# davidea97/Fisher-Nerf-customized

Measured on AMD Instinct MI355X. Metric: candidate-views/sec, higher is better.
Workload: dtype f32

## Files before the change

### fisher-nerf-customized_amd/csrc/fisher_rast.hip

```cpp
#include <hip/hip_runtime.h>
#include <hip/hip_fp16.h>
#include <stdint.h>
#include <stdio.h>
#include <stdlib.h>
#include <string.h>
#include "fr_math.h"
#include "../../include/fisher_rast.h"
#include "fr_internal.h"

#define FR_THREADS 256
#define FR_G_MAX 32
#define FR_MAX_LDS_TILES 4096
#define FR_PART_MIN_DEFAULT 2048
#define FR_SORT_SMALL_KEYS 2048
#define FR_SORT_MID_KEYS 4096
#define FR_SORT_BIG_KEYS 16384
#define FR_VC_MAX 16
#define FR_BATCH 256
#define FR_BWD_BATCH 128

#include <vector>
#include <utility>
static thread_local char g_err[512] = "";
#if defined(FR_ABLATE) || defined(FR_LOOPSTATS)
// ... 33 lines not shown

struct FrParams {
	int P, V, W, H;
	uint32_t gx, gy;
	int T;
	int G;
	float tanfovx, tanfovy, focal_x, focal_y, mod;
	int D, M;
	const float* bg; const float* view; const float* proj; const float* campos;
	const float* w2c;
	const float* means3D; const float* colors; const float* shs; const float* opac;
	const float* scales; const float* rots;
	const float* cov3D;
	float* cov3D_out;
	int* radii;
	FrSplat* splat;
	float* rgb;
	uint8_t* clamped;
	uint32_t* tile_cnt; uint32_t* tile_off; uint32_t* tile_fill;
	uint64_t* keys; long long key_capacity;
	uint32_t* blk_base;
	uint32_t* big_list;
	uint32_t* view_work;
	uint32_t* view_perm;
	int* status;
	int* vis_count;
	int* num_rendered;
	struct FrVisEntry* vis_list;
	uint32_t* vis_n;
	int VC;
	uint32_t tile_cap;
	uint32_t small_max;
	const uint32_t* order;
	int legacy_sort;
	int prefiltered;
	int ablate;
};
#ifdef FR_ABLATE
#define FR_ABL(x) x
#else
#define FR_ABL(x)
#endif

__device__ __forceinline__ float wave_sum(float v)
{
#pragma unroll
// ... 1137 lines not shown
	{
		uint4 en[NB];
#pragma unroll
		for (int b = 0; b < NB; b++)
		{
			const uint32_t e = e0 + b * FR_THREADS + tid;
			en[b] = e < n ? list[e] : make_uint4(0u, 0u, 0u, 0u);
		}
#pragma unroll
		for (int b = 0; b < NB; b++)
		{
			const uint64_t key = ((uint64_t)en[b].y << 32) | en[b].x;
			const uint32_t x0 = en[b].z & 0xffffu, y0 = en[b].z >> 16, x1 = en[b].w & 0xffffu, y1 = en[b].w >> 16;
			for (uint32_t y = y0; y < y1; y++)
				for (uint32_t x = x0; x < x1; x++)
				{
					const uint32_t t = y * p.gx + x;
					p.keys[s_base[t] + atomicAdd(&s_cnt[t], 1u)] = key;
				}
		}
	}
}

__device__ __forceinline__ void fr_tile_of_block(const FrParams& p, uint32_t& tile, int& v)
{
	const uint32_t L = blockIdx.x;
	if ((p.V & 7) == 0)
	{
		const uint32_t xcd = L & 7u, q = L >> 3;
		v = (int)((q / (uint32_t)p.T) * 8u + xcd);
		if (p.view_perm) v = (int)p.view_perm[v];
		tile = q % (uint32_t)p.T;
	}
	else
	{
		v = (int)(L / (uint32_t)p.T);
		tile = L % (uint32_t)p.T;
	}
}

__device__ __forceinline__ void fr_cx(uint64_t& lo, uint64_t& hi)
{
	const uint64_t a = lo, b = hi;
	const bool sw = a > b;
	lo = sw ? b : a; hi = sw ? a : b;
}
template <typename KeyPtr>
__device__ __forceinline__ uint64_t fr_ldk(KeyPtr keys, uint32_t i, uint32_t n) { return i < n ? keys[i] : ~0ull; }
template <typename KeyPtr>
// ... 233 lines not shown
		}
	}
}

template <int K, int NW>
__device__ __forceinline__ void fr_sort_wg_segment(uint64_t* sk, uint64_t* __restrict__ gk, uint32_t n, int tid)
{
	static_assert(NW == 4 || NW == 16, "4 or 16 waves");
	constexpr int RUN = 64 * K;
	const int lane = tid & 63;
	const int w = __builtin_amdgcn_readfirstlane(tid >> 6);
	const uint32_t base = (uint32_t)(w * RUN);
	uint64_t key[K];
#pragma unroll
	for (int r = 0; r < K; r++) { const uint32_t i = base + (uint32_t)(lane * K + r); key[r] = i < n ? gk[i] : ~0ull; }
	uint32_t n_pad = 1;
	while (n_pad < n) n_pad <<= 1;
	fr_wave_stages<K, 6 + FrLog2<K>::value>(key, n_pad, lane);
	fr_wg_stages<K, NW, (NW == 4 ? 2 : 4)>(key, sk, n_pad, w, lane);
#pragma unroll
	for (int r = 0; r < K; r++) { const uint32_t i = base + (uint32_t)(lane * K + r); if (i < n) gk[i] = key[r]; }
}

__global__ __launch_bounds__(FR_THREADS) void k_sort_tiles(FrParams p)
{
	if (p.status[1]) return;
	__shared__ uint64_t skeys[FR_SORT_SMALL_KEYS];
	const int tid = threadIdx.x;
	uint32_t tile; int v;
	fr_tile_of_block(p, tile, v);
	const size_t vt = (size_t)v * p.T + tile;
	const uint32_t n = p.tile_cnt[vt];
	if (n < 2 || n > p.small_max) return;
	uint64_t* gk = p.keys + p.tile_off[vt];
#ifdef FR_AB
	if (p.legacy_sort)
	{
		for (uint32_t i = tid; i < n; i += FR_THREADS) skeys[i] = gk[i];
		__syncthreads();
		fr_bitonic(skeys, n, tid, FR_THREADS);
		for (uint32_t i = tid; i < n; i += FR_THREADS) gk[i] = skeys[i];
		return;
	}
#endif
	if (n <= 512u)
	{
		if (tid >= 64) return;
		if (n <= 64u) fr_sort_wave_segment<1>(gk, n, tid);
		else if (n <= 128u) fr_sort_wave_segment<2>(gk, n, tid);
		else if (n <= 256u) fr_sort_wave_segment<4>(gk, n, tid);
		else fr_sort_wave_segment<8>(gk, n, tid);
		return;
	}
	if (n <= 1024u) fr_sort_wg_segment<4, 4>(skeys, gk, n, tid);
	else fr_sort_wg_segment<8, 4>(skeys, gk, n, tid);
}

#define FR_PART_SAMPLE 512
#define FR_PART_MAXP 64
__global__ __launch_bounds__(FR_THREADS) void k_sort_part(FrParams p, uint32_t part_max)
{
	__shared__ uint64_t skeys[FR_SORT_SMALL_KEYS];
	__shared__ uint64_t s_piv[FR_PART_MAXP];
	__shared__ uint32_t s_cnt[FR_PART_MAXP], s_off[FR_PART_MAXP], s_cur[FR_PART_MAXP];
	__shared__ uint32_t s_next;
	if (p.status[1]) return;
	const int tid = threadIdx.x, lane = tid & 63;
	const uint32_t count = p.big_list[0];
	for (uint32_t b = blockIdx.x; b < count; b += gridDim.x)
	{
		const size_t vt = p.big_list[16 + b];
		const uint32_t n = p.tile_cnt[vt];
		if (n > part_max) continue;
		uint64_t* gk = p.keys + p.tile_off[vt];
		const uint32_t n_al = (n + 63u) & ~63u;
		uint64_t* tmp = gk + n_al;
		const uint32_t NP = n <= 1280u ? 4u : n <= 2560u ? 8u : n <= 5120u ? 16u : n <= 10240u ? 32u : 64u;
		__syncthreads();
		if (tid < FR_PART_MAXP) { s_cnt[tid] = 0u; s_cur[tid] = 0u; }
		if (tid == 0) s_next = 0u;
		if (tid < 64)
		{
			uint64_t key[8];
#pragma unroll
			for (int r = 0; r < 8; r++) key[r] = gk[(uint32_t)(((uint64_t)(uint32_t)(lane * 8 + r) * n) >> 9)];
			fr_wave_stages<8, 9>(key, (uint32_t)FR_PART_SAMPLE, lane);
			const uint32_t step = 64u / NP;
			if (((uint32_t)lane % step) == 0u && lane > 0) s_piv[(uint32_t)lane / step] = key[0];
		}
		__syncthreads();
		auto part_of = [&](uint64_t k) -> uint32_t {
			uint32_t lo = 0u;
			for (uint32_t stepw = NP >> 1; stepw > 0u; stepw >>= 1)
			{
				const uint32_t mid = lo + stepw;
				if (s_piv[mid] <= k) lo = mid;
			}
			return lo;
		};
		constexpr int KB = 8;
		for (uint32_t i0 = 0; i0 < n; i0 += KB * FR_THREADS)
		{
			uint64_t k[KB];
#pragma unroll
			for (int r = 0; r < KB; r++) { const uint32_t i = i0 + r * FR_THREADS + tid; k[r] = i < n ? gk[i] : ~0ull; }
#pragma unroll
			for (int r = 0; r < KB; r++) { const uint32_t i = i0 + r * FR_THREADS + tid; if (i < n) atomicAdd(&s_cnt[part_of(k[r])], 1u); }
		}
		__syncthreads();
		if (tid == 0)
		{
			uint32_t run = 0;
			for (uint32_t q = 0; q < NP; q++) { s_off[q] = run; run += s_cnt[q]; }
		}
		__syncthreads();
		for (uint32_t i0 = 0; i0 < n; i0 += KB * FR_THREADS)
		{
			uint64_t k[KB];
#pragma unroll
			for (int r = 0; r < KB; r++) { const uint32_t i = i0 + r * FR_THREADS + tid; k[r] = i < n ? gk[i] : ~0ull; }
#pragma unroll
			for (int r = 0; r < KB; r++)
			{
				const uint32_t i = i0 + r * FR_THREADS + tid;
				if (i < n) { const uint32_t q = part_of(k[r]); tmp[s_off[q] + atomicAdd(&s_cur[q], 1u)] = k[r]; }
			}
		}
		__syncthreads();
		for (;;)
		{
			uint32_t q = 0;
			if (lane == 0) q = atomicAdd(&s_next, 1u);
			q = (uint32_t)__builtin_amdgcn_readfirstlane((int)q);
			if (q >= NP) break;
			const uint32_t c = s_cnt[q];
			uint64_t* pk = tmp + s_off[q];
			if (c < 2u || c > 512u) continue;
			if (c <= 64u) fr_sort_wave_segment<1>(pk, c, lane);
			else if (c <= 128u) fr_sort_wave_segment<2>(pk, c, lane);
			else if (c <= 256u) fr_sort_wave_segment<4>(pk, c, lane);
			else fr_sort_wave_segment<8>(pk, c, lane);
		}
		__syncthreads();
		for (uint32_t q = 0; q < NP; q++)
		{
			const uint32_t c = s_cnt[q];
			if (c <= 512u) continue;
			uint64_t* pk = tmp + s_off[q];
			if (c <= 1024u) fr_sort_wg_segment<4, 4>(skeys, pk, c, tid);
			else if (c <= (uint32_t)FR_SORT_SMALL_KEYS) fr_sort_wg_segment<8, 4>(skeys, pk, c, tid);
			else fr_bitonic(pk, c, tid, FR_THREADS);
			__syncthreads();
		}
		if (tid == 0) p.tile_off[vt] += n_al;
	}
}

__global__ __launch_bounds__(FR_THREADS) void k_sort_mid_tiles(FrParams p, uint32_t part_max)
{
	if (p.status[1]) return;
	__shared__ uint64_t skeys[FR_SORT_MID_KEYS];
	const int tid = threadIdx.x;
	const uint32_t count = p.big_list[0];
	for (uint32_t b = blockIdx.x; b < count; b += gridDim.x)
	{
		const size_t vt = p.big_list[16 + b];
		const uint32_t n = p.tile_cnt[vt];
		if (n > (uint32_t)FR_SORT_MID_KEYS || n <= part_max) continue;
		uint64_t* gk = p.keys + p.tile_off[vt];
		__syncthreads();
#ifdef FR_AB
		if (p.legacy_sort)
		{
			for (uint32_t i = tid; i < n; i += FR_THREADS) skeys[i] = gk[i];
			__syncthreads();
			fr_bitonic(skeys, n, tid, FR_THREADS);
			for (uint32_t i = tid; i < n; i += FR_THREADS) gk[i] = skeys[i];
// ... 4388 lines not shown
	FrSideStream& ss = sides[which];
	int dev = -1;
	(void)hipGetDevice(&dev);
	if (ss.device != dev)
	{
		if (ss.ok) { (void)hipEventDestroy(ss.fork); (void)hipEventDestroy(ss.join); (void)hipStreamDestroy(ss.stream); }
#ifdef FR_AB
		static const int tile_prio = fr_env_int("FR_TILE_PRIO");
#else
		constexpr int tile_prio = 0;
#endif
		int lo = 0, hi = 0;
		(void)hipDeviceGetStreamPriorityRange(&lo, &hi);
		const int prio = (which == 2 && tile_prio > 0) ? lo : (which == 2 && tile_prio < 0) ? hi : 0;
		ss.ok = hipStreamCreateWithPriority(&ss.stream, hipStreamNonBlocking, prio) == hipSuccess
		     && hipEventCreateWithFlags(&ss.fork, hipEventDisableTiming) == hipSuccess
		     && hipEventCreateWithFlags(&ss.join, hipEventDisableTiming) == hipSuccess;
		ss.device = dev;
		(void)hipGetLastError();
	}
	return ss;
}

struct FrJoinGuard {
	hipStream_t s; FrSideStream* side[2] = { nullptr, nullptr }; int n = 0;
	explicit FrJoinGuard(hipStream_t caller) : s(caller) {}
	void forked(FrSideStream* ss) { side[n++] = ss; }
	int join()
	{
		int rc = FR_OK;
		for (int i = 0; i < n; i++)
		{
			if (hipEventRecord(side[i]->join, side[i]->stream) != hipSuccess || hipStreamWaitEvent(s, side[i]->join, 0) != hipSuccess)
				rc = fr_fail(FR_ELAUNCH, "side stream join failed");
		}
		n = 0;
		return rc;
	}
	~FrJoinGuard() { if (n) { char keep[sizeof(g_err)]; memcpy(keep, g_err, sizeof(keep)); (void)join(); memcpy(g_err, keep, sizeof(keep)); } }
};

struct FrScorerPlan { int columns; bool form_a; FrRecordArgs ra; bool skip_pack = false; bool general = false; bool pose = false; bool view_identity = false; };
template <int C> __global__ void k_pack_static(FrParams p, const float* __restrict__ H_inv, float* __restrict__ packed, float4* __restrict__ mt, float4* __restrict__ grp);
template <int C, bool LIST, bool FORM_A> __global__ void k_fisher_records(FrParams p, FrRecordArgs ra);

static int fr_bin_pipeline(FrParams& p, const fr_gaussians* g, hipStream_t s, const FrScorerPlan* plan = nullptr)
{
	int rc;
	const int P = p.P;
	{
		FrZeroer z;
		z.add(p.tile_cnt, (size_t)p.V * p.T * 4); z.add(p.status, 16); z.add(p.big_list, 64);
		if (p.view_work) z.add(p.view_work, (size_t)p.V * 4);
		if (p.vis_count) z.add(p.vis_count, (size_t)p.V * 4);
		if (p.num_rendered && p.vis_list != nullptr && p.T <= FR_MAX_LDS_TILES) z.add(p.num_rendered, (size_t)p.V * 4);
		z.launch(s);
	}
	const bool multi = p.vis_list != nullptr && p.T <= FR_MAX_LDS_TILES;
	if (g->cov3D_precomp) p.cov3D = g->cov3D_precomp;
	else if (plan && multi) p.cov3D = nullptr;
	else
	{
		hipLaunchKernelGGL(k_cov3d, dim3((P + FR_THREADS - 1) / FR_THREADS), dim3(FR_THREADS), 0, s, P, g->scales, p.mod, g->rotations, p.cov3D_out);
		if ((rc = fr_check_launch("k_cov3d"))) return rc;
		p.cov3D = p.cov3D_out;
	}
	p.G = multi ? fr_pick_G_views(P) : fr_pick_G(P, p.V);
	p.VC = fr_pick_VC(p.T);
	const int per_block = FR_THREADS * p.G;
	dim3 gridP((P + per_block - 1) / per_block, p.V);
	const size_t hist_lds = p.T <= FR_MAX_LDS_TILES ? (size_t)p.T * 4 : 16;
	if (plan && !plan->skip_pack)
	{
		const float* shared_hinv = plan->ra.hinv_stride ? nullptr : plan->ra.H_inv;
		dim3 gp((P + FR_THREADS - 1) / FR_THREADS);
// ... 58 lines not shown
	if ((rc = fr_check_launch("k_scan_tiles"))) return rc;
	if (multi && p.tile_cap) {  }
	else if (multi) hipLaunchKernelGGL(k_scatter_vis, gridP, dim3(FR_THREADS), 2 * hist_lds, s, p);
	else hipLaunchKernelGGL(k_scatter_keys, gridP, dim3(FR_THREADS), 2 * hist_lds, s, p);
	if ((rc = fr_check_launch("k_scatter_keys"))) return rc;
	if (plan && !multi)
	{
		FrSideStream& s2 = fr_side_stream(1);
		const bool forked2 = s2.ok && hipEventRecord(s2.fork, s) == hipSuccess && hipStreamWaitEvent(s2.stream, s2.fork, 0) == hipSuccess;
		hipStream_t rs = forked2 ? s2.stream : s;
		if (plan->form_a) hipLaunchKernelGGL((k_fisher_records<4, false, true>), gridP, dim3(FR_THREADS), 0, rs, p, plan->ra);
		else if (plan->columns == 4) hipLaunchKernelGGL((k_fisher_records<4, false, false>), gridP, dim3(FR_THREADS), 0, rs, p, plan->ra);
		else hipLaunchKernelGGL((k_fisher_records<11, false, false>), gridP, dim3(FR_THREADS), 0, rs, p, plan->ra);
		if (forked2) joins.forked(&s2);
		if ((rc = fr_check_launch("k_fisher_records"))) return rc;
	}
	FrSideStream& side = fr_side_stream();
	const bool part_all = p.tile_cap >= 32768u && fr_debug_mode() != 32;
	const bool want_fork = fr_debug_mode() != 7 && (!multi || p.V >= 8) && !part_all;
	const bool forked = want_fork && side.ok && hipEventRecord(side.fork, s) == hipSuccess && hipStreamWaitEvent(side.stream, side.fork, 0) == hipSuccess;
	const int big_blocks = p.T * p.V < 256 ? p.T * p.V : 256;
	if (forked) joins.forked(&side);
	uint32_t part_max = 0;
	if (p.tile_cap >= 2u * (uint32_t)FR_SORT_SMALL_KEYS + 128u && fr_debug_mode() != 32)
	{
		part_max = p.tile_cap / 2u - 64u;
		if (part_max > 16320u) part_max = 16320u;
	}
	hipLaunchKernelGGL(k_sort_big_tiles, dim3(big_blocks), dim3(1024), 0, forked ? side.stream : s, p, part_max);
	if ((rc = fr_check_launch("k_sort_big_tiles"))) return rc;
	const int mid_blocks = p.T * p.V < 2048 ? p.T * p.V : 2048;
	hipLaunchKernelGGL(k_sort_tiles, dim3(p.T * p.V), dim3(FR_THREADS), 0, s, p);
	if ((rc = fr_check_launch("k_sort_tiles"))) return rc;
	if (part_max)
	{
		hipLaunchKernelGGL(k_sort_part, dim3(mid_blocks), dim3(FR_THREADS), 0, s, p, part_max);
		if ((rc = fr_check_launch("k_sort_part"))) return rc;
	}
	if (part_max < (uint32_t)FR_SORT_MID_KEYS)
	{
		hipLaunchKernelGGL(k_sort_mid_tiles, dim3(mid_blocks), dim3(FR_THREADS), 0, s, p, part_max);
		if ((rc = fr_check_launch("k_sort_mid_tiles"))) return rc;
	}
	return joins.join();
}

static void fr_carve_single(FrParams& p, const FrLayout& L, char* geom, char* bin, char* img)
{
	p.splat = (FrSplat*)(geom + L.splat);
	p.cov3D_out = (float*)(geom + L.cov3D);
	p.rgb = (float*)(geom + L.rgb);
	p.clamped = (uint8_t*)(geom + L.clamped);
	p.tile_cnt = (uint32_t*)(img + L.tile_cnt);
	p.tile_off = (uint32_t*)(img + L.tile_off);
	p.tile_fill = (uint32_t*)(img + L.tile_fill);
	p.status = (int*)(img + L.status);
	p.big_list = (uint32_t*)(img + L.big_list);
	p.blk_base = p.T <= FR_MAX_LDS_TILES ? (uint32_t*)(img + L.blk_base) : nullptr;
	p.keys = (uint64_t*)(bin + L.keys);
}
// ... 382 lines not shown
		b.only_flagged = fallback; b.u_only = 1;
		if (sr) hipLaunchKernelGGL((k_backward_tile<true, false>), grid, block, 0, s, p, b);
		else hipLaunchKernelGGL((k_backward_tile<false, false>), grid, block, 0, s, p, b);
		if ((rc = fr_check_launch("k_backward_tile(flagged)"))) return rc;
	}
	b.dL_dmean2D = dL_dmeans2D; b.dL_dmean2D_b = dL_dmeans2D_features;
	b.dL_dcolors = dL_dcolors; b.colors = g->colors_precomp;
	dim3 gp((P + FR_THREADS - 1) / FR_THREADS);
	if (sr) hipLaunchKernelGGL((k_backward_finish<true, false>), gp, block, 0, s, p, b, (float*)nullptr);
	else hipLaunchKernelGGL((k_backward_finish<false, false>), gp, block, 0, s, p, b, (float*)nullptr);
	return fr_check_launch("k_backward_finish");
}

#ifdef FR_AB
static int fr_debug_mode()
{
	static const int mode = fr_env_int("FR_DEBUG_MODE");
	return mode;
}
#endif

#define FR_MAX_GROUPS 4
struct FrFisherLayout {
	size_t radii, vis_n, splat, recq, slot_idx, packed, mt, grp, big_list, view_work, view_perm, blk_base, cov3D, tile_cnt, tile_off, tile_fill, tile_scores, w2c_inv, status, keys, fallback, seg_T, seg_C, seg_X, seg_list, total;
	size_t PV;
};
static FrFisherLayout fr_fisher_layout(int64_t P, int64_t W, int64_t H, int64_t V, int64_t max_rendered, int columns)
{
	FrFisherLayout L;
	const int64_t T = ((W + 15) / 16) * ((H + 15) / 16);
	size_t o = 0;
	const size_t nblk_v = (size_t)((P + FR_THREADS * fr_pick_G_views(P) - 1) / (FR_THREADS * fr_pick_G_views(P)));
	L.radii = o; o = fr_align(o + (size_t)V * nblk_v * (size_t)(FR_THREADS * fr_pick_G_views(P)) * sizeof(FrVisEntry));
	L.vis_n = o; o = fr_align(o + (size_t)V * nblk_v * 4);
	L.PV = nblk_v * (size_t)(FR_THREADS * fr_pick_G_views(P));
	const size_t VPV = (size_t)V * (L.PV > (size_t)P ? L.PV : (size_t)P);
	L.splat = o; o = fr_align(o + VPV * sizeof(FrSplat));
	L.recq = o; o = fr_align(o + VPV * (columns == 11 ? 208 : 112));
	L.slot_idx = o; o = fr_align(o + VPV * 4);
	L.packed = o; o = fr_align(o + (size_t)P * 4 * (size_t)(columns == 11 ? 32 : 16));
	L.mt = o; o = fr_align(o + (size_t)P * 16);
	L.grp = o; o = fr_align(o + (size_t)((P + FR_THREADS - 1) / FR_THREADS) * 32);
	L.big_list = o; o = fr_align(o + (size_t)(V * T) * 4 + 64 * FR_MAX_GROUPS);
	L.view_work = o; o = fr_align(o + (size_t)V * 4);
	L.view_perm = o; o = fr_align(o + (size_t)V * 4);
	L.blk_base = o; o = fr_align(o + (size_t)V * (size_t)fr_preprocess_blocks(P, V) * (size_t)T * 4);
	L.cov3D = o; o = fr_align(o + (size_t)P * 24);
	L.tile_cnt = o; o = fr_align(o + (size_t)(V * T) * 4);
	L.tile_off = o; o = fr_align(o + (size_t)(V * T) * 4);
	L.tile_fill = o; o = fr_align(o + (size_t)(V * T) * 4);
	L.tile_scores = o; o = fr_align(o + (size_t)(V * T) * 4);
	L.w2c_inv = o; o = fr_align(o + (size_t)V * 64);
	L.status = o; o = fr_align(o + 64);
	const size_t R = (size_t)(max_rendered > 0 ? max_rendered : 1);
	L.keys = o; o = fr_align(o + R * 8);
	L.fallback = o; o = fr_align(o + (size_t)(V * T));
	const size_t seg_tiles = (size_t)(V * T <= FR_SEG_TILES ? V * T : 0);
	L.seg_T = o; o = fr_align(o + FR_SEG_PER_TILE * seg_tiles * FR_THREADS * 4);
	L.seg_C = o; o = fr_align(o + FR_SEG_PER_TILE * seg_tiles * FR_THREADS * 8);
	L.seg_X = o; o = fr_align(o + seg_tiles * FR_THREADS * 8);
	L.seg_list = o; o = fr_align(o + (FR_SEG_PER_TILE * seg_tiles + 1) * 4);
	L.total = o;
	return L;
}

extern "C" int fr_fisher_workspace_layout(int32_t P, int32_t W, int32_t H, int32_t n_views, int64_t max_rendered, int32_t columns, size_t o[8])
{
	if (P < 0 || W <= 0 || H <= 0 || n_views <= 0 || max_rendered < 0 || (columns != 4 && columns != 11) || !o)
		return fr_fail(FR_EINVAL, "fr_fisher_workspace_layout: bad argument");
	const FrFisherLayout L = fr_fisher_layout(P, W, H, n_views, max_rendered, columns);
	o[0] = L.tile_cnt; o[1] = L.tile_off; o[2] = L.keys; o[3] = L.splat; o[4] = L.recq; o[5] = L.tile_scores; o[6] = L.status; o[7] = L.vis_n;
	return FR_OK;
}

extern "C" int fr_init(void)
{
	if (!fr_side_stream(0).ok || !fr_side_stream(1).ok || !fr_side_stream(2).ok) return fr_fail(FR_ELAUNCH, "fr_init: could not create the side streams");
	return FR_OK;
}

extern "C" size_t fr_fisher_workspace_bytes(int32_t P, int32_t W, int32_t H, int32_t n_views, int64_t max_rendered, int32_t columns)
{
	if (P < 0 || W <= 0 || H <= 0 || n_views <= 0 || max_rendered < 0 || (columns != 4 && columns != 11)) return 0;
	return fr_fisher_layout(P, W, H, n_views, max_rendered, columns).total;
}

static void fr_launch_fisher_v3(FrParams& p, FrFisherArgs f, float4* recq, hipStream_t s)
{
	hipEvent_t ev0 = nullptr, ev1 = nullptr;
	if (g_prof_on)
	{
		(void)hipEventCreate(&ev0); (void)hipEventCreate(&ev1);
		(void)hipEventRecord(ev0, s);
	}
// ... 120 lines not shown
	if (!workspace || workspace_bytes < L.total) return fr_fail(FR_ENOSPACE, "fr_fisher_views: workspace smaller than fr_fisher_workspace_bytes()");
	char* ws = (char*)workspace;
	FrParams p;
	fr_fill_params(p, cfg, g, V);
	p.prefiltered = 0;
	p.w2c = fc->w2c;
	if (fc->poses_are_c2w)
	{
		float* inv = (float*)(ws + L.w2c_inv);
		hipLaunchKernelGGL(k_invert_poses, dim3((V + 63) / 64), dim3(64), 0, s, V, fc->w2c, inv);
		if ((rc = fr_check_launch("k_invert_poses"))) return rc;
		p.w2c = inv;
	}
	p.radii = (int*)(ws + L.radii);
	p.vis_list = (FrVisEntry*)(ws + L.radii);
	p.vis_n = (uint32_t*)(ws + L.vis_n);
	p.splat = (FrSplat*)(ws + L.splat);
	p.cov3D_out = (float*)(ws + L.cov3D);
	p.tile_cnt = (uint32_t*)(ws + L.tile_cnt);
	p.tile_off = (uint32_t*)(ws + L.tile_off);
	p.tile_fill = (uint32_t*)(ws + L.tile_fill);
	p.status = (int*)(ws + L.status);
	p.big_list = (uint32_t*)(ws + L.big_list);
	const bool deal = (V & 7) == 0 && V <= 1024 && fr_debug_mode() != 27;
	p.view_work = deal ? (uint32_t*)(ws + L.view_work) : nullptr;
	p.view_perm = deal ? (uint32_t*)(ws + L.view_perm) : nullptr;
	p.blk_base = (uint32_t*)(ws + L.blk_base);
	p.keys = (uint64_t*)(ws + L.keys);
	p.key_capacity = max_rendered;
	if (fc->tile_capacity < 0) return fr_fail(FR_EINVAL, "fr_fisher_views: negative tile_capacity");
	if (fc->tile_capacity > 0)
	{
		const long long need = (long long)V * p.T * (long long)fc->tile_capacity;
		if (need > max_rendered || need >= (1ll << 32)) return fr_fail(FR_EINVAL, "fr_fisher_views: n_views * tiles * tile_capacity exceeds max_rendered (or 2^32)");
		const long long nblk_c = (P + FR_THREADS * fr_pick_G_views(P) - 1) / (FR_THREADS * fr_pick_G_views(P));
		const bool slots_fit = nblk_c * FR_THREADS * fr_pick_G_views(P) < (1ll << 28);
		if (p.gx <= 255u && p.gy <= 63u && slots_fit && fr_debug_mode() != 8 && fr_debug_mode() != 24 && fr_debug_mode() != 20) p.tile_cap = (uint32_t)fc->tile_capacity;
	}
	p.vis_count = fc->out_vis_count;
	p.num_rendered = fc->out_num_rendered;
	FrFisherArgs f;
	f.dL = fc->dL_dpix;
	f.dL_img = fc->dL_dpix_image; f.dL_stride = fc->dL_image_view_stride;
	f.H_inv = fc->H_inv; f.hinv_stride = fc->H_inv_view_stride;
	f.out_H = fc->out_H; f.outH_stride = fc->out_H_view_stride;
	f.tile_scores = (float*)(ws + L.tile_scores);
// ... 43 lines not shown
	static thread_local hipEvent_t front_done[FR_MAX_GROUPS] = { nullptr, nullptr, nullptr, nullptr };
	const size_t nblk_v = (size_t)((P + FR_THREADS * fr_pick_G_views(P) - 1) / (FR_THREADS * fr_pick_G_views(P)));
	const size_t cap_v = (size_t)(FR_THREADS * fr_pick_G_views(P));
	const size_t rec_view = compact ? L.PV : (size_t)P;
	struct TileJoin {
		hipStream_t s; FrSideStream* side; bool on;
		~TileJoin() { if (on) { (void)hipEventRecord(side->join, side->stream); (void)hipStreamWaitEvent(s, side->join, 0); } }
	} tile_join{ s, &tside, false };
	for (int gi = 0; gi < n_groups; gi++)
	{
		const int per = n_groups > 1 ? ((V / n_groups + 7) / 8) * 8 : V;
		const int v0 = gi * per, Vg = (gi == n_groups - 1) ? V - v0 : per;
		if (Vg <= 0) break;
		FrParams pg = p;
		pg.V = Vg;
		pg.w2c = p.w2c + 16 * (size_t)v0;
		pg.radii = p.radii ? (int*)((char*)p.radii + (size_t)v0 * nblk_v * cap_v * sizeof(FrVisEntry)) : nullptr;
		pg.vis_list = p.vis_list + (size_t)v0 * nblk_v * cap_v;
		pg.vis_n = p.vis_n + (size_t)v0 * nblk_v;
		pg.splat = p.splat + (size_t)v0 * rec_view;
		pg.tile_cnt = p.tile_cnt + (size_t)v0 * p.T; pg.tile_off = p.tile_off + (size_t)v0 * p.T; pg.tile_fill = p.tile_fill + (size_t)v0 * p.T;
		pg.status = p.status + 4 * gi;
		pg.big_list = p.big_list + (size_t)v0 * p.T + 16 * gi;
		if (p.view_perm && (Vg & 7) == 0) { pg.view_work = p.view_work + v0; pg.view_perm = p.view_perm + v0; }
		else { pg.view_work = nullptr; pg.view_perm = nullptr; }
		pg.blk_base = p.blk_base + (size_t)v0 * (size_t)fr_preprocess_blocks(P, V) * (size_t)p.T;
		pg.tile_cap = p.tile_cap;
		const long long k0 = (long long)((__int128)max_rendered * v0 / V), k1 = (long long)((__int128)max_rendered * (v0 + Vg) / V);
		pg.keys = p.keys + k0; pg.key_capacity = k1 - k0;
		pg.vis_count = p.vis_count ? p.vis_count + v0 : nullptr;
		pg.num_rendered = p.num_rendered ? p.num_rendered + v0 : nullptr;
		FrScorerPlan pl = plan;
		pl.skip_pack = gi > 0 || (fc->reuse_static != 0 && compact);
		if (pl.ra.hinv_stride) pl.ra.H_inv = plan.ra.H_inv + (size_t)v0 * plan.ra.hinv_stride;
		pl.ra.recq = plan.ra.recq + (size_t)v0 * rec_view * 4;
		if (pl.ra.comp) pl.ra.comp = plan.ra.comp + (size_t)v0 * L.PV * rstride;
		if (pl.ra.slot_idx) pl.ra.slot_idx = plan.ra.slot_idx + (size_t)v0 * L.PV;
		FrFisherArgs fg = f;
		fg.recA = f.recA + (size_t)v0 * f.ab_view; fg.recQ = f.recQ + (size_t)v0 * f.q_view;
		if (f.slot_idx) fg.slot_idx = f.slot_idx + (size_t)v0 * f.slot_view;
		fg.tile_scores = f.tile_scores + (size_t)v0 * p.T;
		if (f.H_inv && f.hinv_stride) fg.H_inv = f.H_inv + (size_t)v0 * f.hinv_stride;
		if (f.out_H && f.outH_stride) fg.out_H = f.out_H + (size_t)v0 * f.outH_stride;
		if (f.dL_img && f.dL_stride) fg.dL_img = f.dL_img + (size_t)v0 * f.dL_stride;

		if ((rc = fr_bin_pipeline(pg, g, s, (v3 || v3h || v3g) ? &pl : nullptr))) return rc;
// ... 87 lines not shown
		return fr_fail(FR_ENOSPACE, "fr_fisher_pose_views: workspace smaller than fr_fisher_pose_workspace_bytes()");
	char* ws = (char*)workspace;
	FrParams p;
	fr_fill_params(p, cfg, g, V);
	p.prefiltered = 0;
	p.w2c = fc->w2c;
	if (fc->poses_are_c2w)
	{
		float* inv = (float*)(ws + L.w2c_inv);
		hipLaunchKernelGGL(k_invert_poses, dim3((V + 63) / 64), dim3(64), 0, s, V, fc->w2c, inv);
		if ((rc = fr_check_launch("k_invert_poses"))) return rc;
		p.w2c = inv;
	}
	p.radii = (int*)(ws + L.radii);
	p.vis_list = (FrVisEntry*)(ws + L.radii);
	p.vis_n = (uint32_t*)(ws + L.vis_n);
	p.splat = (FrSplat*)(ws + L.splat);
	p.cov3D_out = (float*)(ws + L.cov3D);
	p.tile_cnt = (uint32_t*)(ws + L.tile_cnt);
	p.tile_off = (uint32_t*)(ws + L.tile_off);
	p.tile_fill = (uint32_t*)(ws + L.tile_fill);
	p.status = (int*)(ws + L.status);
	p.big_list = (uint32_t*)(ws + L.big_list);
	const bool deal = (V & 7) == 0 && V <= 1024;
	p.view_work = deal ? (uint32_t*)(ws + L.view_work) : nullptr;
	p.view_perm = deal ? (uint32_t*)(ws + L.view_perm) : nullptr;
	p.blk_base = (uint32_t*)(ws + L.blk_base);
	p.keys = (uint64_t*)(ws + L.keys);
	p.key_capacity = max_rendered;
	if (fc->tile_capacity > 0)
	{
		const long long nblk_c = (P + FR_THREADS * fr_pick_G_views(P) - 1) / (FR_THREADS * fr_pick_G_views(P));
		const bool slots_fit = nblk_c * FR_THREADS * fr_pick_G_views(P) < (1ll << 28);
		if (p.gx <= 255u && p.gy <= 63u && slots_fit) p.tile_cap = (uint32_t)fc->tile_capacity;
	}
	(void)fr_plan_views_c(p.T, fr_pick_VC(p.T), p.tile_cap);
	p.vis_count = fc->out_vis_count;
	p.num_rendered = fc->out_num_rendered;
	p.order = fc->order;
	constexpr int rstride = FrRecStride<4, 3>::value;
	FrScorerPlan plan;
	plan.columns = 4;
	plan.form_a = false;
	plan.pose = true;
	plan.ra.H_inv = nullptr; plan.ra.hinv_stride = 0;
	plan.ra.packed = (const float*)(ws + L.packed); plan.ra.recq = (float4*)(ws + L.recq);
// ... 467 lines not shown
```

### fisher-nerf-customized_amd/fisher_rast/_lib.py

```python
import ctypes
import os

_HERE = os.path.dirname(os.path.abspath(__file__))
SO_PATH = os.environ.get("FISHER_RAST_SO", os.path.join(_HERE, "libfisher_rast.so"))

FR_OK, FR_EINVAL, FR_ELAUNCH, FR_ENOSPACE = 0, 1, 2, 3

_f32p = ctypes.c_void_p


class RasterCfg(ctypes.Structure):
    _fields_ = [
        ("P", ctypes.c_int32),
        ("image_height", ctypes.c_int32),
        ("image_width", ctypes.c_int32),
        ("tanfovx", ctypes.c_float),
        ("tanfovy", ctypes.c_float),
        ("scale_modifier", ctypes.c_float),
        ("sh_degree", ctypes.c_int32),
        ("sh_coeffs", ctypes.c_int32),
        ("prefiltered", ctypes.c_int32),
        ("bg", _f32p),
        ("viewmatrix", _f32p),
        ("projmatrix", _f32p),
# ... 30 lines not shown
        ("dL_image_view_stride", ctypes.c_int64),
        ("tile_capacity", ctypes.c_int32),
        ("poses_are_c2w", ctypes.c_int32),
        ("reuse_static", ctypes.c_int32),
        ("order", ctypes.c_void_p),
        ("view_is_identity", ctypes.c_int32),
    ]


class OccCfg(ctypes.Structure):
    _fields_ = [
        ("grid_w", ctypes.c_int32),
        ("grid_h", ctypes.c_int32),
        ("cell_size", ctypes.c_float),
        ("center_x", ctypes.c_float),
        ("center_z", ctypes.c_float),
        ("height_lower", ctypes.c_float),
        ("height_upper", ctypes.c_float),
        ("far_distance", ctypes.c_float),
    ]


EXPORTS = (
    "fr_version", "fr_last_error", "fr_build_id", "fr_init", "fr_fisher_workspace_layout", "fr_workspace_bytes", "fr_workspace_layout", "fr_mark_visible",
    "fr_forward", "fr_backward", "fr_backward_scratch_bytes", "fr_backward_ws", "fr_forward_pair", "fr_forward_features", "fr_backward_pair", "fr_backward_pair_scratch_bytes", "fr_backward_pair_ws", "fr_fisher_workspace_bytes", "fr_fisher_views",
    "fr_fisher_pose_workspace_bytes", "fr_fisher_pose_workspace_layout", "fr_fisher_pose_views",
    "fr_densify_stats", "fr_densify_masks", "fr_prune_mask", "fr_knn_workspace_bytes", "fr_knn_dist2", "fr_spatial_order_workspace_bytes", "fr_spatial_order", "fr_profile_enable", "fr_profile_fetch",
    "fr_occ_workspace_bytes", "fr_occ_update", "fr_occ_freespace", "fr_occ_frontiers", "fr_occ_erode", "fr_occ_cells_of",
    "fr_occ_ring_candidates", "fr_occ_free_candidates",
)

_lib = None

_CSRC = os.path.join(os.path.dirname(_HERE), "csrc")
_INCLUDE = os.path.join(os.path.dirname(os.path.dirname(_HERE)), "include")
SOURCES = [os.path.join(_CSRC, n) for n in ("fisher_rast.hip", "fisher_occ.hip", "fr_math.h", "fr_internal.h")] + \
          [os.path.join(_INCLUDE, n) for n in ("fisher_rast.h", "fisher_occ.h")]


def source_hash():
    import hashlib
    h = hashlib.sha256()
    for f in SOURCES:
        if not os.path.exists(f):
            return None
        h.update(open(f, "rb").read())
    return h.hexdigest()[:16]


class FisherRastError(RuntimeError):
    pass


def load():
    global _lib
    if _lib is not None:
        return _lib
    if not os.path.exists(SO_PATH):
        raise FisherRastError(
            f"{SO_PATH} is missing: the HIP extension has not been built "
            "(run `python -c \"import __graft_entry__ as g; g.build()\"` at the repo root). "
            "There is no CPU fallback for this path.")
    import torch
    lib = ctypes.CDLL(SO_PATH)
    for name in EXPORTS:
        if not hasattr(lib, name):
            raise FisherRastError(f"{SO_PATH} does not export {name}")
    lib.fr_version.restype = ctypes.c_int
    lib.fr_last_error.restype = ctypes.c_char_p
    lib.fr_build_id.restype = ctypes.c_char_p
    lib.fr_init.restype = ctypes.c_int
    lib.fr_fisher_workspace_layout.restype = ctypes.c_int
    lib.fr_fisher_workspace_layout.argtypes = [ctypes.c_int32, ctypes.c_int32, ctypes.c_int32, ctypes.c_int32,
                                               ctypes.c_int64, ctypes.c_int32, ctypes.POINTER(ctypes.c_size_t)]
    want = source_hash()
    got = lib.fr_build_id().decode().split(":")[-1]
    if "FISHER_RAST_SO" not in os.environ and want is not None and got != want:
        raise FisherRastError(f"{SO_PATH} was built from other sources (build id {got}, sources {want}): "
                              "run `python -c \"import __graft_entry__ as g; g.build()\"`")
    lib.fr_workspace_bytes.restype = ctypes.c_int
    lib.fr_workspace_bytes.argtypes = [ctypes.c_int32, ctypes.c_int32, ctypes.c_int32, ctypes.c_int64,
                                       ctypes.POINTER(ctypes.c_size_t)]
    lib.fr_workspace_layout.restype = ctypes.c_int
    lib.fr_workspace_layout.argtypes = [ctypes.c_int32, ctypes.c_int32, ctypes.c_int32, ctypes.c_int64,
                                        ctypes.POINTER(ctypes.c_size_t)]
    lib.fr_mark_visible.restype = ctypes.c_int
    lib.fr_mark_visible.argtypes = [ctypes.c_int32, _f32p, _f32p, _f32p, ctypes.c_void_p, ctypes.c_void_p]
    lib.fr_forward.restype = ctypes.c_int
    lib.fr_forward.argtypes = [ctypes.POINTER(RasterCfg), ctypes.POINTER(Gaussians),
                               ctypes.c_void_p, ctypes.c_void_p, ctypes.c_int64, ctypes.c_void_p,
                               _f32p, _f32p, ctypes.c_void_p, ctypes.c_void_p, ctypes.c_void_p]
    lib.fr_backward.restype = ctypes.c_int
    lib.fr_backward.argtypes = [ctypes.POINTER(RasterCfg), ctypes.POINTER(Gaussians), ctypes.c_void_p,
                                ctypes.c_void_p, ctypes.c_void_p, ctypes.c_void_p,
                                _f32p, ctypes.c_int32] + [_f32p] * 9 + [ctypes.c_void_p]
    lib.fr_backward_scratch_bytes.restype = ctypes.c_size_t
    lib.fr_backward_scratch_bytes.argtypes = [ctypes.c_int32] * 4 + [ctypes.c_int64]
# ... 88 lines not shown
```

### include/fisher_rast.h

```cpp
#ifndef FISHER_RAST_H_INCLUDED
#define FISHER_RAST_H_INCLUDED

#include <stddef.h>
#include <stdint.h>

#ifdef __cplusplus
extern "C" {
#endif

#define FR_VERSION 100

enum {
	FR_OK = 0,
	FR_EINVAL = 1,
	FR_ELAUNCH = 2,
	FR_ENOSPACE = 3
};

#define FR_STATUS_WORDS 4

typedef void* fr_stream_t;

typedef struct fr_raster_cfg {
	int32_t P;
// ... 84 lines not shown
	const float* w2c;
	const float* H_inv;
	int64_t H_inv_view_stride;
	float* out_scores;
	float* out_H;
	int64_t out_H_view_stride;
	int32_t* out_vis_count;
	int32_t* out_num_rendered;
	const float* dL_dpix_image;
	int64_t dL_image_view_stride;
	int32_t tile_capacity;
	int32_t poses_are_c2w;
	int32_t reuse_static;
	const uint32_t* order;
	int32_t view_is_identity;
} fr_fisher_cfg;

size_t fr_spatial_order_workspace_bytes(int32_t P);
int fr_spatial_order(int32_t P, const float* means3D, uint32_t* order_out, void* workspace, size_t workspace_bytes, fr_stream_t stream);

size_t fr_fisher_workspace_bytes(int32_t P, int32_t W, int32_t H, int32_t n_views, int64_t max_rendered, int32_t columns);
int fr_fisher_workspace_layout(int32_t P, int32_t W, int32_t H, int32_t n_views, int64_t max_rendered, int32_t columns,
                               size_t offsets[8]);

int fr_fisher_views(const fr_raster_cfg* cfg, const fr_gaussians* g, const fr_fisher_cfg* cfg_f,
                    void* workspace, size_t workspace_bytes, int64_t max_rendered,
                    int32_t* status, fr_stream_t stream);

size_t fr_fisher_pose_workspace_bytes(int32_t P, int32_t W, int32_t H, int32_t n_views, int64_t max_rendered);
int fr_fisher_pose_workspace_layout(int32_t P, int32_t W, int32_t H, int32_t n_views, int64_t max_rendered, size_t offsets[9]);
int fr_fisher_pose_views(const fr_raster_cfg* cfg, const fr_gaussians* g, const fr_fisher_cfg* cfg_f, float* out_pose_H,
                         void* workspace, size_t workspace_bytes, int64_t max_rendered, int32_t* status, fr_stream_t stream);


int fr_densify_stats(int32_t P, const int32_t* radii, const float* grad_means2D, float* max_2D_radius,
                     float* means2D_gradient_accum, float* denom, uint8_t* seen, fr_stream_t stream);

int fr_densify_masks(int32_t P, const float* means2D_gradient_accum, const float* denom, const float* log_scales,
                     int32_t scale_cols, float grad_thresh, float clone_max_scale, float split_min_scale,
                     uint8_t* to_clone, uint8_t* to_split, fr_stream_t stream);

int fr_prune_mask(int32_t P, const float* logit_opacities, const float* log_scales, int32_t scale_cols,
                  float opacity_thresh, float big_thresh, uint8_t* to_remove, fr_stream_t stream);


size_t fr_knn_workspace_bytes(int32_t P);
// ... 12 lines not shown
```

Baseline: 46060.

## Merge short-tile sort into partition kernel and sort partitions in separate wave kernel

The separate short-tile sort launch is folded into the partition kernel: extra blocks beyond a CU-scaled count sort the short tiles. Mid-size partitions are no longer sorted serially by the waves of the block that partitioned them. Their offsets are appended to a global list and sorted one per wave in a new k_sort_parts kernel, spreading the work across the whole GPU. Pivot sampling now uses all four waves, and the partition prefix sum uses a wave scan. The cost is an extra kernel launch, extra workspace for the partition list, and global atomics.

```diff
diff --git a/fisher-nerf-customized_amd/csrc/fisher_rast.hip b/fisher-nerf-customized_amd/csrc/fisher_rast.hip
--- a/fisher-nerf-customized_amd/csrc/fisher_rast.hip
+++ b/fisher-nerf-customized_amd/csrc/fisher_rast.hip
@@ -79,6 +79,7 @@
 	uint32_t* blk_base;
 	uint32_t* big_list;
 	uint32_t* view_work;
+	uint32_t* part_list;
 	uint32_t* view_perm;
 	int* status;
 	int* vis_count;
@@ -1262,9 +1263,9 @@
 	}
 }
 
-__device__ __forceinline__ void fr_tile_of_block(const FrParams& p, uint32_t& tile, int& v)
-{
-	const uint32_t L = blockIdx.x;
+__device__ __forceinline__ void fr_tile_of_block(const FrParams& p, uint32_t& tile, int& v, uint32_t first = 0u)
+{
+	const uint32_t L = blockIdx.x - first;
 	if ((p.V & 7) == 0)
 	{
 		const uint32_t xcd = L & 7u, q = L >> 3;
@@ -1544,13 +1545,11 @@
 	for (int r = 0; r < K; r++) { const uint32_t i = base + (uint32_t)(lane * K + r); if (i < n) gk[i] = key[r]; }
 }
 
-__global__ __launch_bounds__(FR_THREADS) void k_sort_tiles(FrParams p)
-{
-	if (p.status[1]) return;
-	__shared__ uint64_t skeys[FR_SORT_SMALL_KEYS];
+__device__ __forceinline__ void fr_sort_short_list(const FrParams& p, uint64_t* skeys, uint32_t first)
+{
 	const int tid = threadIdx.x;
 	uint32_t tile; int v;
-	fr_tile_of_block(p, tile, v);
+	fr_tile_of_block(p, tile, v, first);
 	const size_t vt = (size_t)v * p.T + tile;
 	const uint32_t n = p.tile_cnt[vt];
 	if (n < 2 || n > p.small_max) return;
@@ -1578,37 +1577,46 @@
 	else fr_sort_wg_segment<8, 4>(skeys, gk, n, tid);
 }
 
+__global__ __launch_bounds__(FR_THREADS) void k_sort_tiles(FrParams p)
+{
+	if (p.status[1]) return;
+	__shared__ uint64_t skeys[FR_SORT_SMALL_KEYS];
+	fr_sort_short_list(p, skeys, 0u);
+}
+
 #define FR_PART_SAMPLE 512
 #define FR_PART_MAXP 64
-__global__ __launch_bounds__(FR_THREADS) void k_sort_part(FrParams p, uint32_t part_max)
+__global__ __launch_bounds__(FR_THREADS) void k_sort_split(FrParams p, uint32_t part_max, uint32_t split_blocks)
 {
 	__shared__ uint64_t skeys[FR_SORT_SMALL_KEYS];
 	__shared__ uint64_t s_piv[FR_PART_MAXP];
 	__shared__ uint32_t s_cnt[FR_PART_MAXP], s_off[FR_PART_MAXP], s_cur[FR_PART_MAXP];
-	__shared__ uint32_t s_next;
+	__shared__ uint32_t s_over;
 	if (p.status[1]) return;
+	if (blockIdx.x >= split_blocks) { fr_sort_short_list(p, skeys, split_blocks); return; }
 	const int tid = threadIdx.x, lane = tid & 63;
 	const uint32_t count = p.big_list[0];
-	for (uint32_t b = blockIdx.x; b < count; b += gridDim.x)
+	for (uint32_t b = blockIdx.x; b < count; b += split_blocks)
 	{
 		const size_t vt = p.big_list[16 + b];
 		const uint32_t n = p.tile_cnt[vt];
 		if (n > part_max) continue;
-		uint64_t* gk = p.keys + p.tile_off[vt];
+		const uint32_t toff = p.tile_off[vt];
+		uint64_t* gk = p.keys + toff;
 		const uint32_t n_al = (n + 63u) & ~63u;
 		uint64_t* tmp = gk + n_al;
 		const uint32_t NP = n <= 1280u ? 4u : n <= 2560u ? 8u : n <= 5120u ? 16u : n <= 10240u ? 32u : 64u;
 		__syncthreads();
 		if (tid < FR_PART_MAXP) { s_cnt[tid] = 0u; s_cur[tid] = 0u; }
-		if (tid == 0) s_next = 0u;
-		if (tid < 64)
-		{
-			uint64_t key[8];
-#pragma unroll
-			for (int r = 0; r < 8; r++) key[r] = gk[(uint32_t)(((uint64_t)(uint32_t)(lane * 8 + r) * n) >> 9)];
-			fr_wave_stages<8, 9>(key, (uint32_t)FR_PART_SAMPLE, lane);
-			const uint32_t step = 64u / NP;
-			if (((uint32_t)lane % step) == 0u && lane > 0) s_piv[(uint32_t)lane / step] = key[0];
+		{
+			const int w = __builtin_amdgcn_readfirstlane(tid >> 6);
+			uint64_t key[2];
+#pragma unroll
+			for (int r = 0; r < 2; r++) key[r] = gk[(uint32_t)(((uint64_t)(uint32_t)(w * 128 + lane * 2 + r) * n) >> 9)];
+			fr_wave_stages<2, 7>(key, (uint32_t)FR_PART_SAMPLE, lane);
+			fr_wg_stages<2, 4, 2>(key, skeys, (uint32_t)FR_PART_SAMPLE, w, lane);
+			const uint32_t pos = (uint32_t)(w * 128 + lane * 2), step = (uint32_t)FR_PART_SAMPLE / NP;
+			if (pos % step == 0u && pos > 0u) s_piv[pos / step] = key[0];
 		}
 		__syncthreads();
 		auto part_of = [&](uint64_t k) -> uint32_t {
@@ -1630,10 +1638,25 @@
 			for (int r = 0; r < KB; r++) { const uint32_t i = i0 + r * FR_THREADS + tid; if (i < n) atomicAdd(&s_cnt[part_of(k[r])], 1u); }
 		}
 		__syncthreads();
-		if (tid == 0)
-		{
-			uint32_t run = 0;
-			for (uint32_t q = 0; q < NP; q++) { s_off[q] = run; run += s_cnt[q]; }
+		if (tid < 64)
+		{
+			const uint32_t c = (uint32_t)lane < NP ? s_cnt[lane] : 0u;
+			uint32_t run = c;
+#pragma unroll
+			for (int d = 1; d < 64; d <<= 1) { const uint32_t t = __shfl_up(run, d, 64); if (lane >= d) run += t; }
+			s_off[lane] = run - c;
+			const bool item = c >= 2u && c <= 512u;
+			const unsigned long long items = __ballot(item);
+			const unsigned long long over = __ballot(c > 512u);
+			uint32_t base = 0u;
+			if (lane == 0)
+			{
+				if (items) base = atomicAdd(&p.part_list[0], (uint32_t)__popcll(items));
+				s_over = over != 0ull;
+			}
+			base = (uint32_t)__builtin_amdgcn_readfirstlane((int)base);
+			if (item)
+				((uint2*)(p.part_list + 16))[base + (uint32_t)__popcll(items & ((1ull << lane) - 1ull))] = make_uint2(toff + n_al + (run - c), c);
 		}
 		__syncthreads();
 		for (uint32_t i0 = 0; i0 < n; i0 += KB * FR_THREADS)
@@ -1648,21 +1671,8 @@
 				if (i < n) { const uint32_t q = part_of(k[r]); tmp[s_off[q] + atomicAdd(&s_cur[q], 1u)] = k[r]; }
 			}
 		}
-		__syncthreads();
-		for (;;)
-		{
-			uint32_t q = 0;
-			if (lane == 0) q = atomicAdd(&s_next, 1u);
-			q = (uint32_t)__builtin_amdgcn_readfirstlane((int)q);
-			if (q >= NP) break;
-			const uint32_t c = s_cnt[q];
-			uint64_t* pk = tmp + s_off[q];
-			if (c < 2u || c > 512u) continue;
-			if (c <= 64u) fr_sort_wave_segment<1>(pk, c, lane);
-			else if (c <= 128u) fr_sort_wave_segment<2>(pk, c, lane);
-			else if (c <= 256u) fr_sort_wave_segment<4>(pk, c, lane);
-			else fr_sort_wave_segment<8>(pk, c, lane);
-		}
+		if (tid == 0) p.tile_off[vt] = toff + n_al;
+		if (!s_over) continue;
 		__syncthreads();
 		for (uint32_t q = 0; q < NP; q++)
 		{
@@ -1674,7 +1684,25 @@
 			else fr_bitonic(pk, c, tid, FR_THREADS);
 			__syncthreads();
 		}
-		if (tid == 0) p.tile_off[vt] += n_al;
+	}
+}
+
+__global__ __launch_bounds__(FR_THREADS) void k_sort_parts(FrParams p)
+{
+	if (p.status[1]) return;
+	const int lane = threadIdx.x & 63;
+	const uint32_t count = p.part_list[0];
+	const uint2* __restrict__ parts = (const uint2*)(p.part_list + 16);
+	const uint32_t waves = gridDim.x * (uint32_t)(FR_THREADS / 64);
+	for (uint32_t i = blockIdx.x * (uint32_t)(FR_THREADS / 64) + (threadIdx.x >> 6); i < count; i += waves)
+	{
+		const uint2 d = parts[i];
+		uint64_t* pk = p.keys + (uint32_t)__builtin_amdgcn_readfirstlane((int)d.x);
+		const uint32_t c = (uint32_t)__builtin_amdgcn_readfirstlane((int)d.y);
+		if (c <= 64u) fr_sort_wave_segment<1>(pk, c, lane);
+		else if (c <= 128u) fr_sort_wave_segment<2>(pk, c, lane);
+		else if (c <= 256u) fr_sort_wave_segment<4>(pk, c, lane);
+		else fr_sort_wave_segment<8>(pk, c, lane);
 	}
 }
 
@@ -6109,6 +6137,20 @@
 	return ss;
 }
 
+static int fr_cu_count()
+{
+	static thread_local int cus = 0, device = -1;
+	int dev = -1;
+	(void)hipGetDevice(&dev);
+	if (device != dev || cus <= 0)
+	{
+		if (hipDeviceGetAttribute(&cus, hipDeviceAttributeMultiprocessorCount, dev) != hipSuccess || cus <= 0) cus = 256;
+		device = dev;
+		(void)hipGetLastError();
+	}
+	return cus;
+}
+
 struct FrJoinGuard {
 	hipStream_t s; FrSideStream* side[2] = { nullptr, nullptr }; int n = 0;
 	explicit FrJoinGuard(hipStream_t caller) : s(caller) {}
@@ -6138,6 +6180,7 @@
 	{
 		FrZeroer z;
 		z.add(p.tile_cnt, (size_t)p.V * p.T * 4); z.add(p.status, 16); z.add(p.big_list, 64);
+		if (p.part_list) z.add(p.part_list, 4);
 		if (p.view_work) z.add(p.view_work, (size_t)p.V * 4);
 		if (p.vis_count) z.add(p.vis_count, (size_t)p.V * 4);
 		if (p.num_rendered && p.vis_list != nullptr && p.T <= FR_MAX_LDS_TILES) z.add(p.num_rendered, (size_t)p.V * 4);
@@ -6242,7 +6285,7 @@
 	const int big_blocks = p.T * p.V < 256 ? p.T * p.V : 256;
 	if (forked) joins.forked(&side);
 	uint32_t part_max = 0;
-	if (p.tile_cap >= 2u * (uint32_t)FR_SORT_SMALL_KEYS + 128u && fr_debug_mode() != 32)
+	if (p.part_list && p.tile_cap >= 2u * (uint32_t)FR_SORT_SMALL_KEYS + 128u && fr_debug_mode() != 32)
 	{
 		part_max = p.tile_cap / 2u - 64u;
 		if (part_max > 16320u) part_max = 16320u;
@@ -6250,12 +6293,23 @@
 	hipLaunchKernelGGL(k_sort_big_tiles, dim3(big_blocks), dim3(1024), 0, forked ? side.stream : s, p, part_max);
 	if ((rc = fr_check_launch("k_sort_big_tiles"))) return rc;
 	const int mid_blocks = p.T * p.V < 2048 ? p.T * p.V : 2048;
-	hipLaunchKernelGGL(k_sort_tiles, dim3(p.T * p.V), dim3(FR_THREADS), 0, s, p);
-	if ((rc = fr_check_launch("k_sort_tiles"))) return rc;
 	if (part_max)
 	{
-		hipLaunchKernelGGL(k_sort_part, dim3(mid_blocks), dim3(FR_THREADS), 0, s, p, part_max);
-		if ((rc = fr_check_launch("k_sort_part"))) return rc;
+		uint32_t split_blocks = (4u * (uint32_t)fr_cu_count()) & ~7u;
+		if (split_blocks < 8u) split_blocks = 8u;
+		if (split_blocks > (uint32_t)(p.T * p.V)) split_blocks = (uint32_t)(p.T * p.V);
+		FR_AB_ONLY({ const int e = fr_env_int("FR_SPLIT_BLOCKS"); if (e >= 8 && e <= 8192) split_blocks = (uint32_t)e & ~7u; })
+		hipLaunchKernelGGL(k_sort_split, dim3(split_blocks + (uint32_t)(p.T * p.V)), dim3(FR_THREADS), 0, s, p, part_max, split_blocks);
+		if ((rc = fr_check_launch("k_sort_split"))) return rc;
+		uint32_t part_blocks = 8u * (uint32_t)fr_cu_count();
+		FR_AB_ONLY({ const int e = fr_env_int("FR_PART_BLOCKS"); if (e >= 1 && e <= 65536) part_blocks = (uint32_t)e; })
+		hipLaunchKernelGGL(k_sort_parts, dim3(part_blocks), dim3(FR_THREADS), 0, s, p);
+		if ((rc = fr_check_launch("k_sort_parts"))) return rc;
+	}
+	else
+	{
+		hipLaunchKernelGGL(k_sort_tiles, dim3(p.T * p.V), dim3(FR_THREADS), 0, s, p);
+		if ((rc = fr_check_launch("k_sort_tiles"))) return rc;
 	}
 	if (part_max < (uint32_t)FR_SORT_MID_KEYS)
 	{
@@ -6684,7 +6738,7 @@
 
 #define FR_MAX_GROUPS 4
 struct FrFisherLayout {
-	size_t radii, vis_n, splat, recq, slot_idx, packed, mt, grp, big_list, view_work, view_perm, blk_base, cov3D, tile_cnt, tile_off, tile_fill, tile_scores, w2c_inv, status, keys, fallback, seg_T, seg_C, seg_X, seg_list, total;
+	size_t radii, vis_n, splat, recq, slot_idx, packed, mt, grp, big_list, part_list, view_work, view_perm, blk_base, cov3D, tile_cnt, tile_off, tile_fill, tile_scores, w2c_inv, status, keys, fallback, seg_T, seg_C, seg_X, seg_list, total;
 	size_t PV;
 };
 static FrFisherLayout fr_fisher_layout(int64_t P, int64_t W, int64_t H, int64_t V, int64_t max_rendered, int columns)
@@ -6722,6 +6776,7 @@
 	L.seg_C = o; o = fr_align(o + FR_SEG_PER_TILE * seg_tiles * FR_THREADS * 8);
 	L.seg_X = o; o = fr_align(o + seg_tiles * FR_THREADS * 8);
 	L.seg_list = o; o = fr_align(o + (FR_SEG_PER_TILE * seg_tiles + 1) * 4);
+	L.part_list = o; o = fr_align(o + (size_t)(V * T) * FR_PART_MAXP * 8 + 64 * FR_MAX_GROUPS);
 	L.total = o;
 	return L;
 }
@@ -6732,6 +6787,14 @@
 		return fr_fail(FR_EINVAL, "fr_fisher_workspace_layout: bad argument");
 	const FrFisherLayout L = fr_fisher_layout(P, W, H, n_views, max_rendered, columns);
 	o[0] = L.tile_cnt; o[1] = L.tile_off; o[2] = L.keys; o[3] = L.splat; o[4] = L.recq; o[5] = L.tile_scores; o[6] = L.status; o[7] = L.vis_n;
+	return FR_OK;
+}
+
+extern "C" int fr_fisher_part_list_offset(int32_t P, int32_t W, int32_t H, int32_t n_views, int64_t max_rendered, int32_t columns, size_t* offset)
+{
+	if (P < 0 || W <= 0 || H <= 0 || n_views <= 0 || max_rendered < 0 || (columns != 4 && columns != 11) || !offset)
+		return fr_fail(FR_EINVAL, "fr_fisher_part_list_offset: bad argument");
+	*offset = fr_fisher_layout(P, W, H, n_views, max_rendered, columns).part_list;
 	return FR_OK;
 }
 
@@ -6898,6 +6961,7 @@
 	p.tile_fill = (uint32_t*)(ws + L.tile_fill);
 	p.status = (int*)(ws + L.status);
 	p.big_list = (uint32_t*)(ws + L.big_list);
+	p.part_list = (uint32_t*)(ws + L.part_list);
 	const bool deal = (V & 7) == 0 && V <= 1024 && fr_debug_mode() != 27;
 	p.view_work = deal ? (uint32_t*)(ws + L.view_work) : nullptr;
 	p.view_perm = deal ? (uint32_t*)(ws + L.view_perm) : nullptr;
@@ -6987,6 +7051,7 @@
 		pg.tile_cnt = p.tile_cnt + (size_t)v0 * p.T; pg.tile_off = p.tile_off + (size_t)v0 * p.T; pg.tile_fill = p.tile_fill + (size_t)v0 * p.T;
 		pg.status = p.status + 4 * gi;
 		pg.big_list = p.big_list + (size_t)v0 * p.T + 16 * gi;
+		pg.part_list = p.part_list + (size_t)v0 * p.T * (2 * FR_PART_MAXP) + 16 * gi;
 		if (p.view_perm && (Vg & 7) == 0) { pg.view_work = p.view_work + v0; pg.view_perm = p.view_perm + v0; }
 		else { pg.view_work = nullptr; pg.view_perm = nullptr; }
 		pg.blk_base = p.blk_base + (size_t)v0 * (size_t)fr_preprocess_blocks(P, V) * (size_t)p.T;
@@ -7120,6 +7185,7 @@
 	p.tile_fill = (uint32_t*)(ws + L.tile_fill);
 	p.status = (int*)(ws + L.status);
 	p.big_list = (uint32_t*)(ws + L.big_list);
+	p.part_list = (uint32_t*)(ws + L.part_list);
 	const bool deal = (V & 7) == 0 && V <= 1024;
 	p.view_work = deal ? (uint32_t*)(ws + L.view_work) : nullptr;
 	p.view_perm = deal ? (uint32_t*)(ws + L.view_perm) : nullptr;
diff --git a/fisher-nerf-customized_amd/fisher_rast/_lib.py b/fisher-nerf-customized_amd/fisher_rast/_lib.py
--- a/fisher-nerf-customized_amd/fisher_rast/_lib.py
+++ b/fisher-nerf-customized_amd/fisher_rast/_lib.py
@@ -76,7 +76,7 @@
 
 
 EXPORTS = (
-    "fr_version", "fr_last_error", "fr_build_id", "fr_init", "fr_fisher_workspace_layout", "fr_workspace_bytes", "fr_workspace_layout", "fr_mark_visible",
+    "fr_version", "fr_last_error", "fr_build_id", "fr_init", "fr_fisher_workspace_layout", "fr_fisher_part_list_offset", "fr_workspace_bytes", "fr_workspace_layout", "fr_mark_visible",
     "fr_forward", "fr_backward", "fr_backward_scratch_bytes", "fr_backward_ws", "fr_forward_pair", "fr_forward_features", "fr_backward_pair", "fr_backward_pair_scratch_bytes", "fr_backward_pair_ws", "fr_fisher_workspace_bytes", "fr_fisher_views",
     "fr_fisher_pose_workspace_bytes", "fr_fisher_pose_workspace_layout", "fr_fisher_pose_views",
     "fr_densify_stats", "fr_densify_masks", "fr_prune_mask", "fr_knn_workspace_bytes", "fr_knn_dist2", "fr_spatial_order_workspace_bytes", "fr_spatial_order", "fr_profile_enable", "fr_profile_fetch",
@@ -117,8 +117,9 @@
             "There is no CPU fallback for this path.")
     import torch
     lib = ctypes.CDLL(SO_PATH)
+    ab_build = "FISHER_RAST_SO" in os.environ
     for name in EXPORTS:
-        if not hasattr(lib, name):
+        if not hasattr(lib, name) and not ab_build:
             raise FisherRastError(f"{SO_PATH} does not export {name}")
     lib.fr_version.restype = ctypes.c_int
     lib.fr_last_error.restype = ctypes.c_char_p
@@ -127,6 +128,9 @@
     lib.fr_fisher_workspace_layout.restype = ctypes.c_int
     lib.fr_fisher_workspace_layout.argtypes = [ctypes.c_int32, ctypes.c_int32, ctypes.c_int32, ctypes.c_int32,
                                                ctypes.c_int64, ctypes.c_int32, ctypes.POINTER(ctypes.c_size_t)]
+    if hasattr(lib, "fr_fisher_part_list_offset"):
+        lib.fr_fisher_part_list_offset.restype = ctypes.c_int
+        lib.fr_fisher_part_list_offset.argtypes = lib.fr_fisher_workspace_layout.argtypes
     want = source_hash()
     got = lib.fr_build_id().decode().split(":")[-1]
     if "FISHER_RAST_SO" not in os.environ and want is not None and got != want:
diff --git a/include/fisher_rast.h b/include/fisher_rast.h
--- a/include/fisher_rast.h
+++ b/include/fisher_rast.h
@@ -130,6 +130,7 @@
 size_t fr_fisher_workspace_bytes(int32_t P, int32_t W, int32_t H, int32_t n_views, int64_t max_rendered, int32_t columns);
 int fr_fisher_workspace_layout(int32_t P, int32_t W, int32_t H, int32_t n_views, int64_t max_rendered, int32_t columns,
                                size_t offsets[8]);
+int fr_fisher_part_list_offset(int32_t P, int32_t W, int32_t H, int32_t n_views, int64_t max_rendered, int32_t columns, size_t* offset);
 
 int fr_fisher_views(const fr_raster_cfg* cfg, const fr_gaussians* g, const fr_fisher_cfg* cfg_f,
                     void* workspace, size_t workspace_bytes, int64_t max_rendered,
```

Result: faster. 47950, median of 6 (+4.1%).
